# petim0/fly_bProject

Hardware: AMD Instinct MI355X
Metric: env-steps/sec (PPO rollout + update), 8192 envs per GPU (higher is better)
Workload: dtype f32 (optimizer step: fp16x2 operand split; rollout policy + critic: bf16x3 operand split; fp32 accumulate)

## Files before the change

fly_bproject_amd/csrc/fly_body.inc:

```

constexpr int LANES_PER_ENV = 8;
constexpr int BLOCK = 256;
constexpr int ENVS_PER_BLOCK = BLOCK / LANES_PER_ENV;


template <int CTRL>
__device__ __forceinline__ float dpp_f(float x)
{
    return __builtin_bit_cast(float, __builtin_amdgcn_update_dpp(0, __builtin_bit_cast(int, x), CTRL, 0xF, 0xF, true));
}
template <int CTRL>
__device__ __forceinline__ int dpp_i(int x)
{
    return __builtin_amdgcn_update_dpp(0, x, CTRL, 0xF, 0xF, true);
}
__device__ __forceinline__ float row_sum(float x)
{
    x += dpp_f<0xB1>(x);
    x += dpp_f<0x4E>(x);
    x += dpp_f<0x141>(x);
    return x;
}
__device__ __forceinline__ int row_sum_i(int x)
{
// ... 3 lines not shown
    return x;
}
__device__ __forceinline__ float row_get(float x, int src)
{
    return __shfl(x, src, LANES_PER_ENV);
}

__device__ __forceinline__ float dot3(float a0, float a1, float a2, float b0, float b1, float b2)
{
    return fmaf(a0, b0, fmaf(a1, b1, a2 * b2));
}
__device__ __forceinline__ float clampf(float x, float lim) { return fminf(fmaxf(x, -lim), lim); }

struct Root {
    float px, py, pz, qx, qy, qz, qw, vx, vy, vz, wx, wy, wz;
};

__device__ __forceinline__ void quat_rot(const float q[4], float v0, float v1, float v2, float sign, float o[3])
{
    float qw = q[3];
    float s = 2.0f * (qw * qw) - 1.0f;
    float cx = q[1] * v2 - q[2] * v1;
    float cy = q[2] * v0 - q[0] * v2;
    float cz = q[0] * v1 - q[1] * v0;
    float dot = q[0] * v0 + q[1] * v1 + q[2] * v2;
    o[0] = (v0 * s + sign * (cx * qw * 2.0f)) + q[0] * dot * 2.0f;
    o[1] = (v1 * s + sign * (cy * qw * 2.0f)) + q[1] * dot * 2.0f;
    o[2] = (v2 * s + sign * (cz * qw * 2.0f)) + q[2] * dot * 2.0f;
}

__device__ __forceinline__ float py_mod(float a, float b)
{
    float m = fmodf(a, b);
    if (m != 0.0f && ((b < 0.0f) != (m < 0.0f))) m += b;
    return m;
}

struct RootObs {
    float vl[3], wl[3], yaw, roll, pitch, ang, up_proj, heading_proj, pot;
};

__device__ __forceinline__ RootObs root_obs(const FlyConfig* __restrict__ c, const Root& r)
{
    RootObs o;
    const float two_pi = 6.28318530717958647692f;
    float t0 = c->target[0] - r.px, t1 = c->target[1] - r.py, t2 = 0.0f;
    float nrm = sqrtf(t0 * t0 + t1 * t1 + t2 * t2);
    o.pot = -nrm / c->dt;
    float dn = nrm < 1e-9f ? 1e-9f : nrm;
    float d0 = t0 / dn, d1 = t1 / dn, d2 = t2 / dn;
    float x1 = r.qx, y1 = r.qy, z1 = r.qz, w1 = r.qw;
    float x2 = -0.0f, y2 = -0.0f, z2 = -0.0f, w2 = 1.0f;
    float ww = (z1 + x1) * (x2 + y2);
    float yy = (w1 - y1) * (w2 + z2);
    float zz = (w1 + y1) * (w2 - z2);
    float xx = ww + yy + zz;
    float qq = 0.5f * (xx + (z1 - x1) * (x2 - y2));
    float tq[4];
    tq[3] = qq - ww + (z1 - y1) * (y2 - z2);
    tq[0] = qq - xx + (x1 + w1) * (x2 + w2);
    tq[1] = qq - yy + (w1 - x1) * (y2 + z2);
    tq[2] = qq - zz + (z1 + y1) * (w2 - x2);
    float up[3], hd[3];
// ... 9 lines not shown
    float roll = atan2f(sinr, cosr);
    float sinp = 2.0f * (w * y - z * x);
    float pitch;
    if (fabsf(sinp) >= 1.0f) {
        float sgn = (sinp > 0.0f) ? 1.0f : ((sinp < 0.0f) ? -1.0f : 0.0f);
        pitch = 1.57079632679489661923f * sgn;
    } else {
        pitch = asinf(sinp);
    }
    float siny = 2.0f * (w * z + x * y);
    float cosy = w * w + x * x - y * y - z * z;
    float yaw = atan2f(siny, cosy);
    o.roll = py_mod(roll, two_pi);
    o.pitch = py_mod(pitch, two_pi);
    o.yaw = py_mod(yaw, two_pi);
    float walk = atan2f(c->target[2] - r.pz, c->target[0] - r.px);
    o.ang = walk - o.yaw;
    return o;
}

__device__ __forceinline__ float scale_action(float a, float lo, float hi)
{
    float t = 0.5f * (a + 1.0f);
    t = t * (hi - lo);
    return t + lo;
}

struct FlyRegs {
    Root r;
    float jq[3], jqd[3];
    float pot, prev_pot;
    int rs;
    long progress;
    float dm[FLY_DR_PARAMS];
    uint32_t dk;
};

template <int PH, bool DR = false>
__device__ __forceinline__ void fly_load(FlyRegs& st, const FlyConfig* __restrict__ c, const FlyBuffers& b, const int block)
{
    const int n = c->num_envs;
    const int tid = threadIdx.x;
    const int sub = tid & (LANES_PER_ENV - 1);
    const long e_raw = (long)block * ENVS_PER_BLOCK + tid / LANES_PER_ENV;
    const long e = e_raw < n ? e_raw : (long)(n - 1);
    const bool is_leg = sub < FLY_NUM_LEGS;
    const int j0 = 3 * (is_leg ? sub : 0);
    constexpr bool NEED_ROOT = (PH & (PH_RESET | PH_INTEGRATE | PH_OBS | PH_REWARD)) != 0;
    constexpr bool NEED_DOF = (PH & (PH_RESET | PH_INTEGRATE | PH_OBS)) != 0;
    constexpr bool NEED_POT = (PH & (PH_RESET | PH_OBS | PH_REWARD)) != 0;
    constexpr bool NEED_FLAG = (PH & (PH_RESET | PH_REWARD)) != 0;
// ... 9 lines not shown
    for (int i = 0; i < 3; ++i) { st.jq[i] = 0.0f; st.jqd[i] = 0.0f; }
    if (NEED_DOF && is_leg) {
        const float* dp = b.dof_state + e * (FLY_NUM_DOF * 2) + 2 * j0;
#pragma unroll
        for (int i = 0; i < 3; ++i) { st.jq[i] = dp[2 * i]; st.jqd[i] = dp[2 * i + 1]; }
    }
    st.pot = 0.0f; st.prev_pot = 0.0f;
    if (NEED_POT) { st.pot = b.pot[e]; st.prev_pot = b.prev_pot[e]; }
    st.rs = 0;
    if (NEED_FLAG) st.rs = (int)(b.reset[e] != 0);
    st.progress = 0;
    if (NEED_PROG) st.progress = b.progress[e];
    if constexpr (DR && (PH & (PH_RESET | PH_INTEGRATE)) != 0) dr_load_row(c, e, st.dm, st.dk);
}

template <int PH, bool DR = false>
__device__ __forceinline__ void fly_body(const FlyConfig* __restrict__ c, const float* __restrict__ actions, const FlyBuffers& b,
                                         float* obs_tile, const int block, const FlyRegs& st, FlyRegs* st_out = nullptr,
                                         const float* actions_tile = nullptr)
{

    const int n = c->num_envs;
    const int tid = threadIdx.x;
    const int sub = tid & (LANES_PER_ENV - 1);
    const int env_in_blk = tid / LANES_PER_ENV;
    const long e_raw = (long)block * ENVS_PER_BLOCK + env_in_blk;
    const bool valid = e_raw < n;
    const long e = valid ? e_raw : (long)(n - 1);
    const bool is_leg = sub < FLY_NUM_LEGS;
    const bool is_abd = sub < FLY_NUM_ABDOMEN;
    const int leg = is_leg ? sub : 0;
    const int abd = is_abd ? sub : 0;
    const int j0 = 3 * leg;

    float lo[3], hi[3], pose[3];
#pragma unroll
    for (int i = 0; i < 3; ++i) { lo[i] = c->dof_lo[j0 + i]; hi[i] = c->dof_hi[j0 + i]; pose[i] = c->dof_pose[j0 + i]; }

    Root r = st.r;
    float jq[3] = {st.jq[0], st.jq[1], st.jq[2]}, jqd[3] = {st.jqd[0], st.jqd[1], st.jqd[2]}, jt[3] = {0, 0, 0};
    float pot = st.pot, prev_pot = st.prev_pot;
    int rs = st.rs;
    long progress = st.progress;
    float dm[FLY_DR_PARAMS];
    uint32_t dk = 0;
    bool drew = false;
    if constexpr (DR) {
#pragma unroll
        for (int j = 0; j < FLY_DR_PARAMS; ++j) dm[j] = st.dm[j];
        dk = st.dk;
    }
    float cf[3] = {0, 0, 0};
// ... 9 lines not shown
        const float* tp = b.targets + e * FLY_NUM_DOF + j0;
#pragma unroll
        for (int i = 0; i < 3; ++i) jt[i] = tp[i];
    }
    if (!(PH & (PH_INTEGRATE)) && (PH & (PH_OBS | PH_REWARD))) {
        if (is_leg) {
            const float* fp = b.contact + (e * FLY_NUM_CONTACT + FLY_NUM_ABDOMEN + leg) * 3;
            cf[0] = fp[0]; cf[1] = fp[1]; cf[2] = fp[2];
        }
        if (is_abd) {
            const float* fp = b.contact + (e * FLY_NUM_CONTACT + abd) * 3;
            cfa[0] = fp[0]; cfa[1] = fp[1]; cfa[2] = fp[2];
        }
    }

    const bool reset_after = c->reset_after_sim != 0;

    auto do_reset = [&]() {
        if (rs) {
            r.px = 0.0f; r.py = 0.0f; r.pz = c->start_height; r.qx = 0.0f; r.qy = 0.0f; r.qz = 0.0f; r.qw = 1.0f;
            r.vx = r.vy = r.vz = r.wx = r.wy = r.wz = 0.0f;
#pragma unroll
            for (int i = 0; i < 3; ++i) { jq[i] = is_leg ? pose[i] : 0.0f; jqd[i] = 0.0f; }
            float tx = c->target[0] - 0.0f, ty = c->target[1] - 0.0f;
            float nrm = sqrtf(__fadd_rn(__fadd_rn(__fmul_rn(tx, tx), __fmul_rn(ty, ty)), 0.0f));
            float p = -nrm / c->dt;
            prev_pot = p; pot = p;
            rs = 0; progress = 0;
            if constexpr (DR) {
                dr_draw(c, (uint32_t)e, dk, dm);
                dk += 1u;
                drew = true;
            }
        }
    };

    if ((PH & PH_RESET) && !(reset_after && (PH & PH_INTEGRATE))) do_reset();

    if (PH & PH_INTEGRATE) {
        const int nsub = c->substeps;
        const float h = c->dt / (float)nsub;
        const float kp = DR ? __fmul_rn(c->kp, dm[0]) : c->kp, kd = DR ? __fmul_rn(c->kd, dm[1]) : c->kd;
        const float eff = DR ? __fmul_rn(c->effort, dm[2]) : c->effort, vmax = c->vmax, Jinv = 1.0f / c->joint_inertia;
        const float minv = 1.0f / (DR ? __fmul_rn(c->mass, dm[3]) : c->mass), g = DR ? __fmul_rn(c->gravity, dm[5]) : c->gravity;
        const float I0 = DR ? __fmul_rn(c->inertia[0], dm[3]) : c->inertia[0];
        const float I1 = DR ? __fmul_rn(c->inertia[1], dm[3]) : c->inertia[1];
        const float I2 = DR ? __fmul_rn(c->inertia[2], dm[3]) : c->inertia[2];
        const float I0inv = 1.0f / I0, I1inv = 1.0f / I1, I2inv = 1.0f / I2;
        const float vlim = c->max_lin_vel, wlim = c->max_ang_vel;
        const float kc = c->kc, cd = c->cdamp, mu = DR ? __fmul_rn(c->mu, dm[4]) : c->mu, cv = c->cvisc;
        const float Lf = c->femur_len, Lt = c->tibia_len;
        const float ld = 1.0f - h * c->lin_damp, ad = 1.0f - h * c->ang_damp;
        const float att0 = c->leg_attach[leg][0], att1 = c->leg_attach[leg][1], att2 = c->leg_attach[leg][2];
        const float azim = c->leg_azimuth[leg], sg = c->leg_sigma[leg];
        const float ab0 = c->abdomen_pts[abd][0], ab1 = c->abdomen_pts[abd][1], ab2 = c->abdomen_pts[abd][2];
        const float al0 = c->alpha0, be0 = c->beta0;
        const float kc_leg = is_leg ? kc : 0.0f, kc_abd = is_abd ? kc : 0.0f;

        for (int s = 0; s < nsub; ++s) {
#pragma unroll
            for (int i = 0; i < 3; ++i) {
                float tau = fmaf(kp, jt[i] - jq[i], -(kd * jqd[i]));
                tau = fminf(fmaxf(tau, -eff), eff);
                float v = fmaf(h * Jinv, tau, jqd[i]);
                v = fminf(fmaxf(v, -vmax), vmax);
                float x = fmaf(h, v, jq[i]);
                if (x < lo[i]) { x = lo[i]; v = fmaxf(v, 0.0f); }
                if (x > hi[i]) { x = hi[i]; v = fminf(v, 0.0f); }
                jq[i] = x; jqd[i] = v;
            }
            const float qx = r.qx, qy = r.qy, qz = r.qz, qw = r.qw;
            const float R00 = fmaf(-2.0f, fmaf(qy, qy, qz * qz), 1.0f), R01 = 2.0f * fmaf(qx, qy, -(qz * qw)), R02 = 2.0f * fmaf(qx, qz, qy * qw);
            const float R10 = 2.0f * fmaf(qx, qy, qz * qw), R11 = fmaf(-2.0f, fmaf(qx, qx, qz * qz), 1.0f), R12 = 2.0f * fmaf(qy, qz, -(qx * qw));
            const float R20 = 2.0f * fmaf(qx, qz, -(qy * qw)), R21 = 2.0f * fmaf(qy, qz, qx * qw), R22 = fmaf(-2.0f, fmaf(qx, qx, qy * qy), 1.0f);
            float psi = fmaf(sg, jq[0] - pose[0], azim);
            float al = al0 + (jq[1] - pose[1]);
            float gm = al + be0 + (jq[2] - pose[2]);
            float psid = sg * jqd[0], ald = jqd[1], gmd = ald + jqd[2];
            const float sp = __sinf(psi), cp = __cosf(psi);
// ... 40 lines not shown
            float wby = dot3(R01, R11, R21, r.wx, r.wy, r.wz);
            float wbz = dot3(R02, R12, R22, r.wx, r.wy, r.wz);
            float tbx = dot3(R00, R10, R20, Tx, Ty, Tz);
            float tby = dot3(R01, R11, R21, Tx, Ty, Tz);
            float tbz = dot3(R02, R12, R22, Tx, Ty, Tz);
            float ax = (tbx - fmaf(wby * I2, wbz, -(wbz * I1 * wby))) * I0inv;
            float ay = (tby - fmaf(wbz * I0, wbx, -(wbx * I2 * wbz))) * I1inv;
            float az = (tbz - fmaf(wbx * I1, wby, -(wby * I0 * wbx))) * I2inv;
            wbx = clampf(fmaf(h, ax, wbx) * ad, wlim);
            wby = clampf(fmaf(h, ay, wby) * ad, wlim);
            wbz = clampf(fmaf(h, az, wbz) * ad, wlim);
            r.wx = dot3(R00, R01, R02, wbx, wby, wbz);
            r.wy = dot3(R10, R11, R12, wbx, wby, wbz);
            r.wz = dot3(R20, R21, R22, wbx, wby, wbz);
            r.px = fmaf(h, r.vx, r.px); r.py = fmaf(h, r.vy, r.py); r.pz = fmaf(h, r.vz, r.pz);
            const float hh = 0.5f * h;
            float nqx = fmaf(hh, fmaf(r.wx, qw, fmaf(r.wy, qz, -(r.wz * qy))), qx);
            float nqy = fmaf(hh, fmaf(-r.wx, qz, fmaf(r.wy, qw, r.wz * qx)), qy);
            float nqz = fmaf(hh, fmaf(r.wx, qy, fmaf(-r.wy, qx, r.wz * qw)), qz);
            float nqw = fmaf(hh, -fmaf(r.wx, qx, fmaf(r.wy, qy, r.wz * qz)), qw);
            float inv = __builtin_amdgcn_rsqf(fmaf(nqx, nqx, fmaf(nqy, nqy, fmaf(nqz, nqz, nqw * nqw))));
            r.qx = nqx * inv; r.qy = nqy * inv; r.qz = nqz * inv; r.qw = nqw * inv;
        }
    }

    if ((PH & PH_RESET) && reset_after && (PH & PH_INTEGRATE)) do_reset();

    float touching_f = 0.0f;
    float obs_act[3] = {0, 0, 0};
    float z_obs = 0.0f, heading_proj = 0.0f;
    if (PH & PH_OBS) {
        prev_pot = pot;
        RootObs ro = root_obs(c, r);
        pot = ro.pot;
        float* row = obs_tile + env_in_blk * FLY_NUM_OBS;
        if (sub == LANES_PER_ENV - 1) {
            row[0] = r.pz; row[1] = ro.vl[0]; row[2] = ro.vl[1]; row[3] = ro.vl[2];
            row[4] = ro.wl[0]; row[5] = ro.wl[1]; row[6] = ro.wl[2];
            row[7] = ro.yaw; row[8] = ro.roll; row[9] = ro.ang; row[10] = ro.up_proj; row[11] = ro.heading_proj;
            row[66] = ro.pitch;
        }
        z_obs = r.pz; heading_proj = ro.heading_proj;
        if (is_leg) {
            const float vs = c->dof_vel_scale;
#pragma unroll
            for (int i = 0; i < 3; ++i) {
                float u = __fsub_rn(__fsub_rn(__fmul_rn(2.0f, jq[i]), hi[i]), lo[i]) / __fsub_rn(hi[i], lo[i]);
                row[12 + j0 + i] = u;
                row[30 + j0 + i] = __fmul_rn(jqd[i], vs);
                row[48 + j0 + i] = jt[i];
                obs_act[i] = jt[i];
            }
            float ssum = __fadd_rn(__fadd_rn(cf[0], cf[1]), cf[2]);
            touching_f = ssum > 0.0f ? 1.0f : 0.0f;
            row[67 + leg] = touching_f;
        }
        __syncthreads();
        const long tile_base = (long)block * ENVS_PER_BLOCK * FLY_NUM_OBS;
        const long total = (long)n * FLY_NUM_OBS;
// ... 10 lines not shown
        }
    } else if (PH & PH_REWARD) {
        const float* row = b.obs + e * FLY_NUM_OBS;
        z_obs = row[0]; heading_proj = row[11];
        if (is_leg) {
#pragma unroll
            for (int i = 0; i < 3; ++i) obs_act[i] = row[48 + j0 + i];
        }
    }

    if (PH & PH_PROGRESS) progress += 1;

    float reward = 0.0f;
    if (PH & PH_REWARD) {
        if (progress == 0) progress = 1;
        const float uw = c->up_weight, hw = c->heading_weight;
        float elec = 0.0f, acost = 0.0f;
        int lim = 0, touching = 0;
        if (is_leg) {
#pragma unroll
            for (int i = 0; i < 3; ++i) {
                acost += jt[i] * jt[i];
                elec += fabsf(__fsub_rn(jt[i], obs_act[i]));
                lim += (obs_act[i] > __fmul_rn(hi[i], 0.9f)) ? 1 : 0;
                lim += (obs_act[i] < __fmul_rn(lo[i], 0.9f)) ? 1 : 0;
            }
            touching = (__fadd_rn(__fadd_rn(cf[0], cf[1]), cf[2]) > 0.0f) ? 1 : 0;
        }
        elec = row_sum(elec); acost = row_sum(acost);
        lim = row_sum_i(lim); touching = row_sum_i(touching);
        float bsum = is_abd ? __fadd_rn(__fadd_rn(cfa[0], cfa[1]), cfa[2]) : 0.0f;
        float abd_sum = 0.0f;
#pragma unroll
        for (int k = 0; k < FLY_NUM_ABDOMEN; ++k) abd_sum = __fadd_rn(abd_sum, row_get(bsum, k));
        const float z = z_obs;
        float heading_r = (heading_proj > 0.8f) ? hw : __fmul_rn(hw, heading_proj) / 0.8f;
        float up_r = 0.0f;
        if (z > 1.4f) up_r = __fadd_rn(up_r, uw);
        if (z < 2.1f) up_r = __fsub_rn(up_r, uw);
        float ori = __fadd_rn(__fmul_rn(r.qz, r.qz), __fmul_rn(r.qw, r.qw));
        float orient_r = (ori > 0.98f) ? uw : 0.0f;
        float leg_r = __fmul_rn((float)touching, 0.1f);
        float progress_r = __fsub_rn(pot, prev_pot);
        float total;
        if (c->reward_mode == 0) {
            total = __fadd_rn(0.5f, __fmul_rn(up_r, orient_r));
            total = __fsub_rn(total, __fmul_rn(c->energy_cost_scale, elec));
            total = __fsub_rn(total, __fmul_rn((float)lim, c->joints_at_limit_cost_scale));
            total = __fadd_rn(total, leg_r);
        } else {
            total = __fadd_rn(__fmul_rn(progress_r, 2.0f), 0.5f);
            total = __fadd_rn(total, __fmul_rn(up_r, orient_r));
            total = __fadd_rn(total, heading_r);
            total = __fsub_rn(total, __fmul_rn(c->actions_cost_scale, acost));
            total = __fsub_rn(total, __fmul_rn(c->energy_cost_scale, elec));
            total = __fsub_rn(total, __fmul_rn((float)lim, c->joints_at_limit_cost_scale));
        }
        const bool dead = (z < c->termination_height) || (z > c->termination_height_up) || (ori < 0.5f) || (abd_sum > 0.0f);
        if (dead) total = c->death_cost;
        if (dead || progress >= (long)c->max_episode_length - 1) rs = 1;
        reward = total;
    }

    if (st_out) {
        st_out->r = r;
#pragma unroll
        for (int i = 0; i < 3; ++i) { st_out->jq[i] = jq[i]; st_out->jqd[i] = jqd[i]; }
        st_out->pot = pot; st_out->prev_pot = prev_pot; st_out->rs = rs; st_out->progress = progress;
        if constexpr (DR) {
#pragma unroll
            for (int j = 0; j < FLY_DR_PARAMS; ++j) st_out->dm[j] = dm[j];
            st_out->dk = dk;
        }
    }
    if (!valid) return;
    if constexpr (DR) {
        if (drew && sub == 0) dr_store_row(c, e, dm, dk);
    }
    if (PH & (PH_SCALE)) {
        if (is_leg) {
            float* tp = b.targets + e * FLY_NUM_DOF + j0;
#pragma unroll
            for (int i = 0; i < 3; ++i) tp[i] = jt[i];
        }
    }
    if (PH & (PH_RESET | PH_INTEGRATE)) {
        if (is_leg) {
            float* dp = b.dof_state + e * (FLY_NUM_DOF * 2) + 2 * j0;
#pragma unroll
            for (int i = 0; i < 3; ++i) { dp[2 * i] = jq[i]; dp[2 * i + 1] = jqd[i]; }
        }
        if (sub == LANES_PER_ENV - 1) {
            float* rp = b.root + e * FLY_ROOT_DIM;
            rp[0] = r.px; rp[1] = r.py; rp[2] = r.pz; rp[3] = r.qx; rp[4] = r.qy; rp[5] = r.qz; rp[6] = r.qw;
            rp[7] = r.vx; rp[8] = r.vy; rp[9] = r.vz; rp[10] = r.wx; rp[11] = r.wy; rp[12] = r.wz;
        }
    }
    if (PH & PH_INTEGRATE) {
        if (is_leg) {
            float* fp = b.contact + (e * FLY_NUM_CONTACT + FLY_NUM_ABDOMEN + leg) * 3;
            fp[0] = cf[0]; fp[1] = cf[1]; fp[2] = cf[2];
        }
        if (is_abd) {
            float* fp = b.contact + (e * FLY_NUM_CONTACT + abd) * 3;
            fp[0] = cfa[0]; fp[1] = cfa[1]; fp[2] = cfa[2];
        }
    }
    if (sub == LANES_PER_ENV - 2) {
        if (PH & (PH_RESET | PH_OBS)) { b.pot[e] = pot; b.prev_pot[e] = prev_pot; }
        if (PH & (PH_RESET | PH_REWARD)) b.reset[e] = (int64_t)rs;
        if (PH & (PH_RESET | PH_REWARD | PH_PROGRESS)) b.progress[e] = (int64_t)progress;
        if (PH & PH_REWARD) {
            b.reward[e] = reward;
            if (b.ep_return) {
                const float er = b.ep_return[e] + reward, el = b.ep_length[e] + 1.0f;
                if (rs) {
                    b.done_return[e] += er; b.done_length[e] += el; b.done_count[e] += 1.0f;
                    b.ep_return[e] = 0.0f; b.ep_length[e] = 0.0f;
                } else {
                    b.ep_return[e] = er; b.ep_length[e] = el;
                }
            }
        }
    }
}
```

fly_bproject_amd/csrc/fly_env.hip:

```cpp
#include <hip/hip_runtime.h>
#include <stdint.h>
#include <type_traits>
#include "flyhip.h"
#include "domain_rand.h"
#include "launch.h"

namespace {

#include "fly_body.inc"

template <int PH>
__global__ __launch_bounds__(BLOCK) void fly_kernel(const FlyConfig* __restrict__ c,
                                                    const float* __restrict__ actions, FlyBuffers b)
{
    __shared__ __attribute__((aligned(16))) float obs_tile[ENVS_PER_BLOCK * FLY_NUM_OBS];
    FlyRegs st;
    fly_load<PH>(st, c, b, blockIdx.x);
    fly_body<PH>(c, actions, b, obs_tile, blockIdx.x, st);
}

template <int PH>
__global__ __launch_bounds__(BLOCK) void fly_dr_kernel(const FlyConfig* __restrict__ c,
                                                       const float* __restrict__ actions, FlyBuffers b)
{
    __shared__ __attribute__((aligned(16))) float obs_tile[ENVS_PER_BLOCK * FLY_NUM_OBS];
    FlyRegs st;
    fly_load<PH, true>(st, c, b, blockIdx.x);
    fly_body<PH, true>(c, actions, b, obs_tile, blockIdx.x, st);
}

inline int grid_for(int n) { return (n + ENVS_PER_BLOCK - 1) / ENVS_PER_BLOCK; }

}

extern "C" hipError_t flyhip_launch_env(int phases, const FlyConfig* dcfg, int n, const float* actions,
                                        const FlyBuffers* b, void* stream, int dr)
{
    constexpr int PH_ALL = PH_SCALE | PH_RESET | PH_INTEGRATE | PH_OBS | PH_PROGRESS | PH_REWARD;
    const dim3 grid(grid_for(n));
    if (dr && (phases & (PH_RESET | PH_INTEGRATE)))
        return with_int<PH_ALL, PH_RESET, PH_INTEGRATE>(phases, [&](auto ph) {
            return launch_kernel<fly_dr_kernel<ph.value>>(grid, BLOCK, 0, stream, dcfg, actions, *b);
        });
// ... 5 lines not shown
```

fly_bproject_amd/csrc/mlp_mfma.hip:

```cpp
#include <hip/hip_runtime.h>
#include <stdint.h>
#include <type_traits>
#include <cstdio>
#include <cstdlib>
#include "flyhip.h"
#include "mlp_layout.h"
#include "obs_norm.h"
#include "domain_rand.h"
#include "launch.h"

namespace {

#include "loss_head.inc"
#include "mlp_gemm.inc"
#include "fs_stamp.inc"
#include "mlp_forward.inc"
#include "mlp_backward.inc"
#include "mlp_grad_w.inc"
#include "mlp_fused_step.inc"
#include "mlp_adam.inc"
#include "fly_body.inc"

template <class Arith>
constexpr int RS_LDS_FLOATS = Arith::FWD_FLOATS > ENVS_PER_BLOCK * FLY_NUM_OBS ? Arith::FWD_FLOATS : ENVS_PER_BLOCK * FLY_NUM_OBS;
// ... 11 lines not shown
    typedef ArithOf<B3> Arith;
    constexpr int ARENA = RS_LDS_FLOATS<Arith>;
    __shared__ __attribute__((aligned(16))) float lds[ARENA + (NORM ? NORM_LDS_FLOATS : 0)];
    float* const norm_tab = NORM ? lds + ARENA : nullptr;
    if (NORM) obs_norm_load(norm_tab, c);
    var_steps -= var_base ? *var_base : 0;
    constexpr int PH_ALL = PH_SCALE | PH_RESET | PH_INTEGRATE | PH_OBS | PH_PROGRESS | PH_REWARD;
    FlyRegs st;
    fly_load<PH_ALL, DR>(st, c, b, blockIdx.x);
    if (NORM) __syncthreads();
    forward_body<Arith, false, false, NORM>(lds, blockIdx.x, 1L << 40, P, PF, x, n, nullptr, v_out, nullptr, nullptr, nullptr, nullptr, eps,
                                            var, act, logp, nullptr, var_steps, var_decay, var_min, norm_tab);
    __builtin_amdgcn_fence(__ATOMIC_RELEASE, "workgroup");
    __builtin_amdgcn_s_waitcnt(0);
    __syncthreads();
    fly_body<PH_ALL, DR>(c, act, b, lds, blockIdx.x, st);
}

__device__ __forceinline__ void store_pose(float* __restrict__ poses, int t, const FlyRegs& nx)
{
    const int sub = threadIdx.x;
    if (sub >= LANES_PER_ENV) return;
    float* p = poses + (long)t * FLY_POSE_FLOATS;
    if (sub < FLY_NUM_LEGS) {
#pragma unroll
        for (int i = 0; i < 3; ++i) p[7 + 3 * sub + i] = nx.jq[i];
    }
    if (sub == LANES_PER_ENV - 1) {
        p[0] = nx.r.px; p[1] = nx.r.py; p[2] = nx.r.pz; p[3] = nx.r.qx; p[4] = nx.r.qy; p[5] = nx.r.qz; p[6] = nx.r.qw;
    }
}
// ... 5 lines not shown
    float var_min, float* __restrict__ act_all, float* __restrict__ logp_all, float* __restrict__ v_ring,
    float* __restrict__ reward_all, int T, const int* __restrict__ rows_applied, int64_t* __restrict__ reset_rows,
    int64_t* __restrict__ progress_rows, float* __restrict__ poses)
{
    typedef ArithOf<B3> Arith;
    constexpr int ARENA = RS_LDS_FLOATS<Arith>;
    __shared__ __attribute__((aligned(16))) float lds[ARENA + 32 + BM * MLP_NACT + (NORM ? NORM_LDS_FLOATS : 0)];
    float* const norm_tab = NORM ? lds + ARENA + 32 + BM * MLP_NACT : nullptr;
    if (NORM) obs_norm_load(norm_tab, c);
    constexpr int PH_ALL = PH_SCALE | PH_RESET | PH_INTEGRATE | PH_OBS | PH_PROGRESS | PH_REWARD;
    float* varcur = lds + ARENA;
    float* acts = B3 ? lds + ARENA + 32 : nullptr;
    if (threadIdx.x < MLP_NACT) varcur[threadIdx.x] = var[threadIdx.x];
    FlyRegs st;
    fly_load<PH_ALL, DR>(st, c, b, blockIdx.x);
    __syncthreads();
    const bool whole = (long)(blockIdx.x + 1) * BM <= n;
    for (int t = 0; t < T; ++t) {
        const float* x = obs_ring + (long)t * n * FLY_NUM_OBS;
        float* act = act_all + (long)t * n * MLP_NACT;
        b.obs = obs_ring + (long)(t + 1) * n * FLY_NUM_OBS;
        b.reward = reward_all + (long)t * n;
        if (reset_rows) { b.reset = reset_rows + (long)t * n; b.progress = progress_rows + (long)t * n; }
        const bool in_lds = B3 && whole;
        forward_body<Arith, false, false, NORM>(lds, blockIdx.x, 1L << 40, P, PF, x, n, nullptr, v_ring + (long)t * n, nullptr, nullptr,
                                                nullptr, nullptr, eps_all + (long)t * n * MLP_NACT, varcur, act, logp_all + (long)t * n,
                                                nullptr, 0, var_decay, var_min, norm_tab, in_lds && t > 0 ? lds : nullptr,
                                                in_lds ? acts : nullptr, B3 && t > 0);
        if (!in_lds) {
            __builtin_amdgcn_fence(__ATOMIC_RELEASE, "workgroup");
            __builtin_amdgcn_s_waitcnt(0);
        }
        __syncthreads();
        FlyRegs nx;
        fly_body<PH_ALL, DR>(c, act, b, lds, blockIdx.x, st, &nx, in_lds ? acts : nullptr);
        if (REC && blockIdx.x == 0) store_pose(poses, t, nx);
        st = nx;
        if (threadIdx.x < MLP_NACT && var_decay > 0.0f) varcur[threadIdx.x] = fmaxf(var_min, varcur[threadIdx.x] - var_decay);
        if (!in_lds) asm volatile("s_waitcnt vmcnt(0)" ::: "memory");
        __syncthreads();
    }
}

template <bool STAMP, bool MULTI, bool REC, bool NORM = false, bool DR = false>
__global__ __launch_bounds__(THREADS, 1) void rollout_all_fs_kernel(
    const FlyConfig* __restrict__ c, FlyBuffers b, const float* __restrict__ P, const u16* __restrict__ PB,
    float* __restrict__ obs_ring, long n, const float* __restrict__ eps_all, const float* __restrict__ var, float var_decay,
    float var_min, float* __restrict__ act_all, float* __restrict__ logp_all, float* __restrict__ v_ring,
    float* __restrict__ reward_all, int T, int64_t* __restrict__ reset_rows, int64_t* __restrict__ progress_rows,
    void* __restrict__ aux)
{
    static_assert(!(STAMP && REC) && !(STAMP && NORM) && !(STAMP && DR), "the stamped diagnostic form neither records, normalises nor randomises");
    unsigned long long* const stamps = static_cast<unsigned long long*>(aux);
    float* const poses = static_cast<float*>(aux);
    extern __shared__ __attribute__((aligned(16))) u16 fr_lds[];
    const FrLds L(fr_lds);
    constexpr int PH_ALL = PH_SCALE | PH_RESET | PH_INTEGRATE | PH_OBS | PH_PROGRESS | PH_REWARD;
    policy_tile_fs_setup(L, P);
    float* const norm_tab = NORM ? reinterpret_cast<float*>(fr_lds) + FR_LDS_BYTES / 4 : nullptr;
    if (NORM) obs_norm_load(norm_tab, c);
    int64_t* const reset0 = b.reset;
    int64_t* const progress0 = b.progress;
    const long ntiles = n / BM;
    long tile = blockIdx.x;
    do {
        unsigned long long* st_tile = STAMP ? stamps + tile * (T + 1) * 8 : nullptr;
        if (threadIdx.x < 32) L.varcur[threadIdx.x] = threadIdx.x < MLP_NACT ? var[threadIdx.x] : 1.0f;
        b.reset = reset0; b.progress = progress0;
        FlyRegs st;
        fly_load<PH_ALL, DR>(st, c, b, (int)tile);
        WeightHeadT<2> w1;
        policy_tile_fs_head(w1, PB);
        __syncthreads();
        if (STAMP && threadIdx.x == 0) st_tile[6] = realtime_cu();
        for (int t = 0; t < T; ++t) {
            stamp<STAMP>(st_tile, 8 * t);
            float* act = act_all + (long)t * n * MLP_NACT;
            b.obs = obs_ring + (long)(t + 1) * n * FLY_NUM_OBS;
            b.reward = reward_all + (long)t * n;
            if (reset_rows) { b.reset = reset_rows + (long)t * n; b.progress = progress_rows + (long)t * n; }
            policy_tile_fs<STAMP, NORM>(L, tile, PB, t == 0 ? obs_ring : nullptr, n, v_ring + (long)t * n, eps_all + (long)t * n * MLP_NACT,
                                        act, logp_all + (long)t * n, w1, STAMP ? st_tile + 8 * t : nullptr, norm_tab);
            stamp<STAMP>(st_tile, 8 * t + 7);
            policy_tile_fs_head(w1, PB);
            FlyRegs nx;
            fly_body<PH_ALL, DR>(c, act, b, L.obs, (int)tile, st, &nx, L.acts);
            if (REC && tile == 0) store_pose(poses, t, nx);
            st = nx;
            if (threadIdx.x < MLP_NACT && var_decay > 0.0f) L.varcur[threadIdx.x] = fmaxf(var_min, L.varcur[threadIdx.x] - var_decay);
            __syncthreads();
        }
        stamp<STAMP>(st_tile, 8 * T);
        if (STAMP && threadIdx.x == 0) st_tile[8 * T + 1] = realtime_cu();
        tile += gridDim.x;
    } while (MULTI && tile < ntiles);
}

}

extern "C" hipError_t flyhip_launch_rollout_all(const FlyConfig* dcfg, const FlyBuffers* b, const float* P, const float* PF,
                                                float* obs_ring, int64_t n, const float* eps_all, const float* var,
                                                float var_decay, float var_min, float* act_all, float* logp_all, float* v_ring,
                                                float* reward_all, int T, const int* rows_applied, const uint16_t* PB,
                                                int64_t* reset_rows, int64_t* progress_rows, void* stream,
                                                unsigned long long* stamps, float* poses, int norm, int dr)
{
// ... 298 lines not shown
```

Baseline: 69.90 million.

## Keep env state and episode stats in registers across rollout steps, hoist config constants

The fused rollout kernels now carry episode return/length statistics, joint targets and contact forces in registers across all T steps, and write the physics state to global memory once at the end instead of every step. Config-derived constants (substep size, inverse masses and inertias, reward weights) are loaded once per block into a pinned register struct rather than re-read from the config pointer each step. The intent is to cut per-step global stores and loads plus scalar config reads. The cost is more register pressure, which may lower occupancy, and intermediate state buffers are no longer current during the rollout.

```diff
diff --git a/fly_bproject_amd/csrc/fly_body.inc b/fly_bproject_amd/csrc/fly_body.inc
--- a/fly_bproject_amd/csrc/fly_body.inc
+++ b/fly_bproject_amd/csrc/fly_body.inc
@@ -41,6 +41,103 @@
 
 struct Root {
     float px, py, pz, qx, qy, qz, qw, vx, vy, vz, wx, wy, wz;
+};
+
+struct FlyLane {
+    float lo[3], hi[3], pose[3];
+    int n, reset_after;
+};
+struct FlyDyn {
+    int nsub;
+    float kp, kd, effort, vmax, mass, gravity, inertia[3], mu;
+    float h, hh, hJinv, minv, Iinv[3], ld, ad;
+    float vlim, wlim, cd, cv, Lf, Lt, al0, be0;
+    float att[3], azim, sg, ab[3];
+    float kc_leg, kc_abd;
+};
+struct FlyTask {
+    int reward_mode, max_episode_length;
+    float dt, target[3], start_height, dof_vel_scale, up_weight, heading_weight;
+    float actions_cost_scale, energy_cost_scale, joints_at_limit_cost_scale, death_cost, termination_height, termination_height_up;
+};
+
+template <bool PIN>
+__device__ __forceinline__ float fly_pin(float x)
+{
+    if constexpr (PIN) asm("" : "+v"(x));
+    return x;
+}
+
+__device__ __forceinline__ void fly_lane(FlyLane& k, const FlyConfig* c, const int leg)
+{
+    const int j0 = 3 * leg;
+#pragma unroll
+    for (int i = 0; i < 3; ++i) { k.lo[i] = c->dof_lo[j0 + i]; k.hi[i] = c->dof_hi[j0 + i]; k.pose[i] = c->dof_pose[j0 + i]; }
+    k.n = c->num_envs; k.reset_after = c->reset_after_sim;
+}
+
+template <bool PIN = false>
+__device__ __forceinline__ FlyDyn fly_dyn(const FlyConfig* c, const int leg, const int abd, const bool is_leg, const bool is_abd)
+{
+    FlyDyn k;
+    auto f = [](float x) { return fly_pin<PIN>(x); };
+    k.nsub = c->substeps;
+    const float h = c->dt / (float)k.nsub, Jinv = 1.0f / c->joint_inertia;
+    k.h = f(h); k.hh = f(0.5f * h); k.hJinv = f(h * Jinv);
+    k.kp = f(c->kp); k.kd = f(c->kd); k.effort = f(c->effort); k.vmax = f(c->vmax); k.mass = f(c->mass); k.gravity = f(c->gravity);
+    k.minv = f(1.0f / c->mass);
+#pragma unroll
+    for (int i = 0; i < 3; ++i) { k.inertia[i] = f(c->inertia[i]); k.Iinv[i] = f(1.0f / c->inertia[i]); }
+    k.vlim = f(c->max_lin_vel); k.wlim = f(c->max_ang_vel);
+    const float kc = c->kc;
+    k.cd = f(c->cdamp); k.mu = f(c->mu); k.cv = f(c->cvisc);
+    k.Lf = f(c->femur_len); k.Lt = f(c->tibia_len);
+    k.ld = f(1.0f - h * c->lin_damp); k.ad = f(1.0f - h * c->ang_damp);
+#pragma unroll
+    for (int i = 0; i < 3; ++i) { k.att[i] = c->leg_attach[leg][i]; k.ab[i] = c->abdomen_pts[abd][i]; }
+    k.azim = c->leg_azimuth[leg]; k.sg = c->leg_sigma[leg];
+    k.al0 = f(c->alpha0); k.be0 = f(c->beta0);
+    k.kc_leg = is_leg ? kc : 0.0f; k.kc_abd = is_abd ? kc : 0.0f;
+    return k;
+}
+
+template <bool PIN = false>
+__device__ __forceinline__ FlyTask fly_task(const FlyConfig* c)
+{
+    FlyTask k;
+    auto f = [](float x) { return fly_pin<PIN>(x); };
+    k.reward_mode = c->reward_mode; k.max_episode_length = c->max_episode_length;
+    k.dt = f(c->dt); k.start_height = f(c->start_height);
+#pragma unroll
+    for (int i = 0; i < 3; ++i) k.target[i] = f(c->target[i]);
+    k.dof_vel_scale = f(c->dof_vel_scale); k.up_weight = f(c->up_weight); k.heading_weight = f(c->heading_weight);
+    k.actions_cost_scale = f(c->actions_cost_scale); k.energy_cost_scale = f(c->energy_cost_scale);
+    k.joints_at_limit_cost_scale = f(c->joints_at_limit_cost_scale); k.death_cost = f(c->death_cost);
+    k.termination_height = f(c->termination_height); k.termination_height_up = f(c->termination_height_up);
+    return k;
+}
+
+struct FlyRead {
+    const FlyConfig* c;
+    __device__ __forceinline__ void lane(FlyLane& k, int leg) const { fly_lane(k, c, leg); }
+    __device__ __forceinline__ FlyDyn dyn(int leg, int abd, bool is_leg, bool is_abd) const { return fly_dyn(c, leg, abd, is_leg, is_abd); }
+    __device__ __forceinline__ FlyTask task() const { return fly_task(c); }
+};
+struct FlyConsts {
+    FlyLane l;
+    FlyDyn d;
+    FlyTask t;
+    __device__ __forceinline__ explicit FlyConsts(const FlyConfig* c)
+    {
+        const int sub = threadIdx.x & (LANES_PER_ENV - 1);
+        const bool is_leg = sub < FLY_NUM_LEGS, is_abd = sub < FLY_NUM_ABDOMEN;
+        fly_lane(l, c, is_leg ? sub : 0);
+        d = fly_dyn<true>(c, is_leg ? sub : 0, is_abd ? sub : 0, is_leg, is_abd);
+        t = fly_task<true>(c);
+    }
+    __device__ __forceinline__ void lane(FlyLane& k, int) const { k = l; }
+    __device__ __forceinline__ const FlyDyn& dyn(int, int, bool, bool) const { return d; }
+    __device__ __forceinline__ const FlyTask& task() const { return t; }
 };
 
 __device__ __forceinline__ void quat_rot(const float q[4], float v0, float v1, float v2, float sign, float o[3])
@@ -67,13 +164,13 @@
     float vl[3], wl[3], yaw, roll, pitch, ang, up_proj, heading_proj, pot;
 };
 
-__device__ __forceinline__ RootObs root_obs(const FlyConfig* __restrict__ c, const Root& r)
+__device__ __forceinline__ RootObs root_obs(const FlyTask& c, const Root& r)
 {
     RootObs o;
     const float two_pi = 6.28318530717958647692f;
-    float t0 = c->target[0] - r.px, t1 = c->target[1] - r.py, t2 = 0.0f;
+    float t0 = c.target[0] - r.px, t1 = c.target[1] - r.py, t2 = 0.0f;
     float nrm = sqrtf(t0 * t0 + t1 * t1 + t2 * t2);
-    o.pot = -nrm / c->dt;
+    o.pot = -nrm / c.dt;
     float dn = nrm < 1e-9f ? 1e-9f : nrm;
     float d0 = t0 / dn, d1 = t1 / dn, d2 = t2 / dn;
     float x1 = r.qx, y1 = r.qy, z1 = r.qz, w1 = r.qw;
@@ -113,7 +210,7 @@
     o.roll = py_mod(roll, two_pi);
     o.pitch = py_mod(pitch, two_pi);
     o.yaw = py_mod(yaw, two_pi);
-    float walk = atan2f(c->target[2] - r.pz, c->target[0] - r.px);
+    float walk = atan2f(c.target[2] - r.pz, c.target[0] - r.px);
     o.ang = walk - o.yaw;
     return o;
 }
@@ -134,6 +231,66 @@
     float dm[FLY_DR_PARAMS];
     uint32_t dk;
 };
+
+struct FlyCarry {
+    float ep_return, ep_length, done_return, done_length, done_count;
+    float jt0, jt1, jt2, cf0, cf1, cf2, cfa0, cfa1, cfa2;
+};
+struct FlyNoCarry {};
+
+template <int PH>
+__device__ __forceinline__ void fly_store_state(const FlyBuffers& b, const long e, const int sub, const float (&jt)[3], const float (&jq)[3],
+                                                const float (&jqd)[3], const Root& r, const float (&cf)[3], const float (&cfa)[3])
+{
+    const bool is_leg = sub < FLY_NUM_LEGS, is_abd = sub < FLY_NUM_ABDOMEN;
+    const int leg = is_leg ? sub : 0, abd = is_abd ? sub : 0, j0 = 3 * leg;
+    if (PH & (PH_SCALE)) {
+        if (is_leg) {
+            float* tp = b.targets + e * FLY_NUM_DOF + j0;
+#pragma unroll
+            for (int i = 0; i < 3; ++i) tp[i] = jt[i];
+        }
+    }
+    if (PH & (PH_RESET | PH_INTEGRATE)) {
+        if (is_leg) {
+            float* dp = b.dof_state + e * (FLY_NUM_DOF * 2) + 2 * j0;
+#pragma unroll
+            for (int i = 0; i < 3; ++i) { dp[2 * i] = jq[i]; dp[2 * i + 1] = jqd[i]; }
+        }
+        if (sub == LANES_PER_ENV - 1) {
+            float* rp = b.root + e * FLY_ROOT_DIM;
+            rp[0] = r.px; rp[1] = r.py; rp[2] = r.pz; rp[3] = r.qx; rp[4] = r.qy; rp[5] = r.qz; rp[6] = r.qw;
+            rp[7] = r.vx; rp[8] = r.vy; rp[9] = r.vz; rp[10] = r.wx; rp[11] = r.wy; rp[12] = r.wz;
+        }
+    }
+    if (PH & PH_INTEGRATE) {
+        if (is_leg) {
+            float* fp = b.contact + (e * FLY_NUM_CONTACT + FLY_NUM_ABDOMEN + leg) * 3;
+            fp[0] = cf[0]; fp[1] = cf[1]; fp[2] = cf[2];
+        }
+        if (is_abd) {
+            float* fp = b.contact + (e * FLY_NUM_CONTACT + abd) * 3;
+            fp[0] = cfa[0]; fp[1] = cfa[1]; fp[2] = cfa[2];
+        }
+    }
+}
+
+template <int PH>
+__device__ __forceinline__ void fly_store_carried(const FlyBuffers& b, const int block, const int n, const FlyRegs& st, const FlyCarry& cy)
+{
+    const int sub = threadIdx.x & (LANES_PER_ENV - 1);
+    const long e = (long)block * ENVS_PER_BLOCK + threadIdx.x / LANES_PER_ENV;
+    if (e >= n) return;
+    const float jt[3] = {cy.jt0, cy.jt1, cy.jt2}, jq[3] = {st.jq[0], st.jq[1], st.jq[2]}, jqd[3] = {st.jqd[0], st.jqd[1], st.jqd[2]};
+    const float cf[3] = {cy.cf0, cy.cf1, cy.cf2}, cfa[3] = {cy.cfa0, cy.cfa1, cy.cfa2};
+    fly_store_state<PH>(b, e, sub, jt, jq, jqd, st.r, cf, cfa);
+    if (sub != LANES_PER_ENV - 2) return;
+    b.pot[e] = st.pot; b.prev_pot[e] = st.prev_pot;
+    if (b.ep_return) {
+        b.ep_return[e] = cy.ep_return; b.ep_length[e] = cy.ep_length;
+        b.done_return[e] = cy.done_return; b.done_length[e] = cy.done_length; b.done_count[e] = cy.done_count;
+    }
+}
 
 template <int PH, bool DR = false>
 __device__ __forceinline__ void fly_load(FlyRegs& st, const FlyConfig* __restrict__ c, const FlyBuffers& b, const int block)
@@ -173,28 +330,41 @@
     if constexpr (DR && (PH & (PH_RESET | PH_INTEGRATE)) != 0) dr_load_row(c, e, st.dm, st.dk);
 }
 
-template <int PH, bool DR = false>
-__device__ __forceinline__ void fly_body(const FlyConfig* __restrict__ c, const float* __restrict__ actions, const FlyBuffers& b,
-                                         float* obs_tile, const int block, const FlyRegs& st, FlyRegs* st_out = nullptr,
-                                         const float* actions_tile = nullptr)
-{
-
+__device__ __forceinline__ void fly_load_carry(FlyCarry& cy, const FlyConfig* __restrict__ c, const FlyBuffers& b, const int block)
+{
     const int n = c->num_envs;
+    const long e_raw = (long)block * ENVS_PER_BLOCK + threadIdx.x / LANES_PER_ENV;
+    const long e = e_raw < n ? e_raw : (long)(n - 1);
+    cy = FlyCarry{};
+    if (b.ep_return) {
+        cy.ep_return = b.ep_return[e]; cy.ep_length = b.ep_length[e];
+        cy.done_return = b.done_return[e]; cy.done_length = b.done_length[e]; cy.done_count = b.done_count[e];
+    }
+}
+
+template <int PH, bool DR = false, class Consts, class Carry = FlyNoCarry>
+__device__ __forceinline__ void fly_body(const FlyConfig* __restrict__ c, const Consts& K, const float* __restrict__ actions,
+                                         const FlyBuffers& b, float* obs_tile, const int block, const FlyRegs& st,
+                                         FlyRegs* st_out = nullptr, const float* actions_tile = nullptr, Carry* cy = nullptr)
+{
+    constexpr bool CARRY = std::is_same<Carry, FlyCarry>::value;
+
     const int tid = threadIdx.x;
     const int sub = tid & (LANES_PER_ENV - 1);
     const int env_in_blk = tid / LANES_PER_ENV;
-    const long e_raw = (long)block * ENVS_PER_BLOCK + env_in_blk;
-    const bool valid = e_raw < n;
-    const long e = valid ? e_raw : (long)(n - 1);
     const bool is_leg = sub < FLY_NUM_LEGS;
     const bool is_abd = sub < FLY_NUM_ABDOMEN;
     const int leg = is_leg ? sub : 0;
     const int abd = is_abd ? sub : 0;
     const int j0 = 3 * leg;
-
-    float lo[3], hi[3], pose[3];
-#pragma unroll
-    for (int i = 0; i < 3; ++i) { lo[i] = c->dof_lo[j0 + i]; hi[i] = c->dof_hi[j0 + i]; pose[i] = c->dof_pose[j0 + i]; }
+    FlyLane kl;
+    K.lane(kl, leg);
+    const int n = kl.n;
+    const long e_raw = (long)block * ENVS_PER_BLOCK + env_in_blk;
+    const bool valid = e_raw < n;
+    const long e = valid ? e_raw : (long)(n - 1);
+
+    const float (&lo)[3] = kl.lo, (&hi)[3] = kl.hi, (&pose)[3] = kl.pose;
 
     Root r = st.r;
     float jq[3] = {st.jq[0], st.jq[1], st.jq[2]}, jqd[3] = {st.jqd[0], st.jqd[1], st.jqd[2]}, jt[3] = {0, 0, 0};
@@ -234,17 +404,18 @@
         }
     }
 
-    const bool reset_after = c->reset_after_sim != 0;
+    const bool reset_after = kl.reset_after != 0;
 
     auto do_reset = [&]() {
         if (rs) {
-            r.px = 0.0f; r.py = 0.0f; r.pz = c->start_height; r.qx = 0.0f; r.qy = 0.0f; r.qz = 0.0f; r.qw = 1.0f;
+            const FlyTask& k = K.task();
+            r.px = 0.0f; r.py = 0.0f; r.pz = k.start_height; r.qx = 0.0f; r.qy = 0.0f; r.qz = 0.0f; r.qw = 1.0f;
             r.vx = r.vy = r.vz = r.wx = r.wy = r.wz = 0.0f;
 #pragma unroll
             for (int i = 0; i < 3; ++i) { jq[i] = is_leg ? pose[i] : 0.0f; jqd[i] = 0.0f; }
-            float tx = c->target[0] - 0.0f, ty = c->target[1] - 0.0f;
+            float tx = k.target[0] - 0.0f, ty = k.target[1] - 0.0f;
             float nrm = sqrtf(__fadd_rn(__fadd_rn(__fmul_rn(tx, tx), __fmul_rn(ty, ty)), 0.0f));
-            float p = -nrm / c->dt;
+            float p = -nrm / k.dt;
             prev_pot = p; pot = p;
             rs = 0; progress = 0;
             if constexpr (DR) {
@@ -258,31 +429,32 @@
     if ((PH & PH_RESET) && !(reset_after && (PH & PH_INTEGRATE))) do_reset();
 
     if (PH & PH_INTEGRATE) {
-        const int nsub = c->substeps;
-        const float h = c->dt / (float)nsub;
-        const float kp = DR ? __fmul_rn(c->kp, dm[0]) : c->kp, kd = DR ? __fmul_rn(c->kd, dm[1]) : c->kd;
-        const float eff = DR ? __fmul_rn(c->effort, dm[2]) : c->effort, vmax = c->vmax, Jinv = 1.0f / c->joint_inertia;
-        const float minv = 1.0f / (DR ? __fmul_rn(c->mass, dm[3]) : c->mass), g = DR ? __fmul_rn(c->gravity, dm[5]) : c->gravity;
-        const float I0 = DR ? __fmul_rn(c->inertia[0], dm[3]) : c->inertia[0];
-        const float I1 = DR ? __fmul_rn(c->inertia[1], dm[3]) : c->inertia[1];
-        const float I2 = DR ? __fmul_rn(c->inertia[2], dm[3]) : c->inertia[2];
-        const float I0inv = 1.0f / I0, I1inv = 1.0f / I1, I2inv = 1.0f / I2;
-        const float vlim = c->max_lin_vel, wlim = c->max_ang_vel;
-        const float kc = c->kc, cd = c->cdamp, mu = DR ? __fmul_rn(c->mu, dm[4]) : c->mu, cv = c->cvisc;
-        const float Lf = c->femur_len, Lt = c->tibia_len;
-        const float ld = 1.0f - h * c->lin_damp, ad = 1.0f - h * c->ang_damp;
-        const float att0 = c->leg_attach[leg][0], att1 = c->leg_attach[leg][1], att2 = c->leg_attach[leg][2];
-        const float azim = c->leg_azimuth[leg], sg = c->leg_sigma[leg];
-        const float ab0 = c->abdomen_pts[abd][0], ab1 = c->abdomen_pts[abd][1], ab2 = c->abdomen_pts[abd][2];
-        const float al0 = c->alpha0, be0 = c->beta0;
-        const float kc_leg = is_leg ? kc : 0.0f, kc_abd = is_abd ? kc : 0.0f;
+        const FlyDyn& k = K.dyn(leg, abd, is_leg, is_abd);
+        const int nsub = k.nsub;
+        const float h = k.h, hJinv = k.hJinv, hh = k.hh;
+        const float kp = DR ? __fmul_rn(k.kp, dm[0]) : k.kp, kd = DR ? __fmul_rn(k.kd, dm[1]) : k.kd;
+        const float eff = DR ? __fmul_rn(k.effort, dm[2]) : k.effort, vmax = k.vmax;
+        const float minv = DR ? 1.0f / __fmul_rn(k.mass, dm[3]) : k.minv, g = DR ? __fmul_rn(k.gravity, dm[5]) : k.gravity;
+        const float I0 = DR ? __fmul_rn(k.inertia[0], dm[3]) : k.inertia[0];
+        const float I1 = DR ? __fmul_rn(k.inertia[1], dm[3]) : k.inertia[1];
+        const float I2 = DR ? __fmul_rn(k.inertia[2], dm[3]) : k.inertia[2];
+        const float I0inv = DR ? 1.0f / I0 : k.Iinv[0], I1inv = DR ? 1.0f / I1 : k.Iinv[1], I2inv = DR ? 1.0f / I2 : k.Iinv[2];
+        const float vlim = k.vlim, wlim = k.wlim;
+        const float cd = k.cd, mu = DR ? __fmul_rn(k.mu, dm[4]) : k.mu, cv = k.cv;
+        const float Lf = k.Lf, Lt = k.Lt;
+        const float ld = k.ld, ad = k.ad;
+        const float att0 = k.att[0], att1 = k.att[1], att2 = k.att[2];
+        const float azim = k.azim, sg = k.sg;
+        const float ab0 = k.ab[0], ab1 = k.ab[1], ab2 = k.ab[2];
+        const float al0 = k.al0, be0 = k.be0;
+        const float kc_leg = k.kc_leg, kc_abd = k.kc_abd;
 
         for (int s = 0; s < nsub; ++s) {
 #pragma unroll
             for (int i = 0; i < 3; ++i) {
                 float tau = fmaf(kp, jt[i] - jq[i], -(kd * jqd[i]));
                 tau = fminf(fmaxf(tau, -eff), eff);
-                float v = fmaf(h * Jinv, tau, jqd[i]);
+                float v = fmaf(hJinv, tau, jqd[i]);
                 v = fminf(fmaxf(v, -vmax), vmax);
                 float x = fmaf(h, v, jq[i]);
                 if (x < lo[i]) { x = lo[i]; v = fmaxf(v, 0.0f); }
@@ -353,7 +525,6 @@
             r.wy = dot3(R10, R11, R12, wbx, wby, wbz);
             r.wz = dot3(R20, R21, R22, wbx, wby, wbz);
             r.px = fmaf(h, r.vx, r.px); r.py = fmaf(h, r.vy, r.py); r.pz = fmaf(h, r.vz, r.pz);
-            const float hh = 0.5f * h;
             float nqx = fmaf(hh, fmaf(r.wx, qw, fmaf(r.wy, qz, -(r.wz * qy))), qx);
             float nqy = fmaf(hh, fmaf(-r.wx, qz, fmaf(r.wy, qw, r.wz * qx)), qy);
             float nqz = fmaf(hh, fmaf(r.wx, qy, fmaf(-r.wy, qx, r.wz * qw)), qz);
@@ -370,7 +541,8 @@
     float z_obs = 0.0f, heading_proj = 0.0f;
     if (PH & PH_OBS) {
         prev_pot = pot;
-        RootObs ro = root_obs(c, r);
+        const FlyTask& k = K.task();
+        RootObs ro = root_obs(k, r);
         pot = ro.pot;
         float* row = obs_tile + env_in_blk * FLY_NUM_OBS;
         if (sub == LANES_PER_ENV - 1) {
@@ -381,7 +553,7 @@
         }
         z_obs = r.pz; heading_proj = ro.heading_proj;
         if (is_leg) {
-            const float vs = c->dof_vel_scale;
+            const float vs = k.dof_vel_scale;
 #pragma unroll
             for (int i = 0; i < 3; ++i) {
                 float u = __fsub_rn(__fsub_rn(__fmul_rn(2.0f, jq[i]), hi[i]), lo[i]) / __fsub_rn(hi[i], lo[i]);
@@ -422,7 +594,8 @@
     float reward = 0.0f;
     if (PH & PH_REWARD) {
         if (progress == 0) progress = 1;
-        const float uw = c->up_weight, hw = c->heading_weight;
+        const FlyTask& k = K.task();
+        const float uw = k.up_weight, hw = k.heading_weight;
         float elec = 0.0f, acost = 0.0f;
         int lim = 0, touching = 0;
         if (is_leg) {
@@ -451,23 +624,38 @@
         float leg_r = __fmul_rn((float)touching, 0.1f);
         float progress_r = __fsub_rn(pot, prev_pot);
         float total;
-        if (c->reward_mode == 0) {
+        if (k.reward_mode == 0) {
             total = __fadd_rn(0.5f, __fmul_rn(up_r, orient_r));
-            total = __fsub_rn(total, __fmul_rn(c->energy_cost_scale, elec));
-            total = __fsub_rn(total, __fmul_rn((float)lim, c->joints_at_limit_cost_scale));
+            total = __fsub_rn(total, __fmul_rn(k.energy_cost_scale, elec));
+            total = __fsub_rn(total, __fmul_rn((float)lim, k.joints_at_limit_cost_scale));
             total = __fadd_rn(total, leg_r);
         } else {
             total = __fadd_rn(__fmul_rn(progress_r, 2.0f), 0.5f);
             total = __fadd_rn(total, __fmul_rn(up_r, orient_r));
             total = __fadd_rn(total, heading_r);
-            total = __fsub_rn(total, __fmul_rn(c->actions_cost_scale, acost));
-            total = __fsub_rn(total, __fmul_rn(c->energy_cost_scale, elec));
-            total = __fsub_rn(total, __fmul_rn((float)lim, c->joints_at_limit_cost_scale));
-        }
-        const bool dead = (z < c->termination_height) || (z > c->termination_height_up) || (ori < 0.5f) || (abd_sum > 0.0f);
-        if (dead) total = c->death_cost;
-        if (dead || progress >= (long)c->max_episode_length - 1) rs = 1;
+            total = __fsub_rn(total, __fmul_rn(k.actions_cost_scale, acost));
+            total = __fsub_rn(total, __fmul_rn(k.energy_cost_scale, elec));
+            total = __fsub_rn(total, __fmul_rn((float)lim, k.joints_at_limit_cost_scale));
+        }
+        const bool dead = (z < k.termination_height) || (z > k.termination_height_up) || (ori < 0.5f) || (abd_sum > 0.0f);
+        if (dead) total = k.death_cost;
+        if (dead || progress >= (long)k.max_episode_length - 1) rs = 1;
         reward = total;
+    }
+
+    if constexpr (CARRY) {
+        if ((PH & PH_REWARD) && b.ep_return) {
+            const float er = cy->ep_return + reward, el = cy->ep_length + 1.0f;
+            if (rs) {
+                cy->done_return += er; cy->done_length += el; cy->done_count += 1.0f;
+                cy->ep_return = 0.0f; cy->ep_length = 0.0f;
+            } else {
+                cy->ep_return = er; cy->ep_length = el;
+            }
+        }
+        cy->jt0 = jt[0]; cy->jt1 = jt[1]; cy->jt2 = jt[2];
+        cy->cf0 = cf[0]; cy->cf1 = cf[1]; cy->cf2 = cf[2];
+        cy->cfa0 = cfa[0]; cy->cfa1 = cfa[1]; cy->cfa2 = cfa[2];
     }
 
     if (st_out) {
@@ -485,42 +673,14 @@
     if constexpr (DR) {
         if (drew && sub == 0) dr_store_row(c, e, dm, dk);
     }
-    if (PH & (PH_SCALE)) {
-        if (is_leg) {
-            float* tp = b.targets + e * FLY_NUM_DOF + j0;
-#pragma unroll
-            for (int i = 0; i < 3; ++i) tp[i] = jt[i];
-        }
-    }
-    if (PH & (PH_RESET | PH_INTEGRATE)) {
-        if (is_leg) {
-            float* dp = b.dof_state + e * (FLY_NUM_DOF * 2) + 2 * j0;
-#pragma unroll
-            for (int i = 0; i < 3; ++i) { dp[2 * i] = jq[i]; dp[2 * i + 1] = jqd[i]; }
-        }
-        if (sub == LANES_PER_ENV - 1) {
-            float* rp = b.root + e * FLY_ROOT_DIM;
-            rp[0] = r.px; rp[1] = r.py; rp[2] = r.pz; rp[3] = r.qx; rp[4] = r.qy; rp[5] = r.qz; rp[6] = r.qw;
-            rp[7] = r.vx; rp[8] = r.vy; rp[9] = r.vz; rp[10] = r.wx; rp[11] = r.wy; rp[12] = r.wz;
-        }
-    }
-    if (PH & PH_INTEGRATE) {
-        if (is_leg) {
-            float* fp = b.contact + (e * FLY_NUM_CONTACT + FLY_NUM_ABDOMEN + leg) * 3;
-            fp[0] = cf[0]; fp[1] = cf[1]; fp[2] = cf[2];
-        }
-        if (is_abd) {
-            float* fp = b.contact + (e * FLY_NUM_CONTACT + abd) * 3;
-            fp[0] = cfa[0]; fp[1] = cfa[1]; fp[2] = cfa[2];
-        }
-    }
+    if constexpr (!CARRY) fly_store_state<PH>(b, e, sub, jt, jq, jqd, r, cf, cfa);
     if (sub == LANES_PER_ENV - 2) {
-        if (PH & (PH_RESET | PH_OBS)) { b.pot[e] = pot; b.prev_pot[e] = prev_pot; }
+        if (!CARRY && (PH & (PH_RESET | PH_OBS))) { b.pot[e] = pot; b.prev_pot[e] = prev_pot; }
         if (PH & (PH_RESET | PH_REWARD)) b.reset[e] = (int64_t)rs;
         if (PH & (PH_RESET | PH_REWARD | PH_PROGRESS)) b.progress[e] = (int64_t)progress;
         if (PH & PH_REWARD) {
             b.reward[e] = reward;
-            if (b.ep_return) {
+            if (!CARRY && b.ep_return) {
                 const float er = b.ep_return[e] + reward, el = b.ep_length[e] + 1.0f;
                 if (rs) {
                     b.done_return[e] += er; b.done_length[e] += el; b.done_count[e] += 1.0f;
diff --git a/fly_bproject_amd/csrc/fly_env.hip b/fly_bproject_amd/csrc/fly_env.hip
--- a/fly_bproject_amd/csrc/fly_env.hip
+++ b/fly_bproject_amd/csrc/fly_env.hip
@@ -16,7 +16,7 @@
     __shared__ __attribute__((aligned(16))) float obs_tile[ENVS_PER_BLOCK * FLY_NUM_OBS];
     FlyRegs st;
     fly_load<PH>(st, c, b, blockIdx.x);
-    fly_body<PH>(c, actions, b, obs_tile, blockIdx.x, st);
+    fly_body<PH>(c, FlyRead{c}, actions, b, obs_tile, blockIdx.x, st);
 }
 
 template <int PH>
@@ -26,7 +26,7 @@
     __shared__ __attribute__((aligned(16))) float obs_tile[ENVS_PER_BLOCK * FLY_NUM_OBS];
     FlyRegs st;
     fly_load<PH, true>(st, c, b, blockIdx.x);
-    fly_body<PH, true>(c, actions, b, obs_tile, blockIdx.x, st);
+    fly_body<PH, true>(c, FlyRead{c}, actions, b, obs_tile, blockIdx.x, st);
 }
 
 inline int grid_for(int n) { return (n + ENVS_PER_BLOCK - 1) / ENVS_PER_BLOCK; }
diff --git a/fly_bproject_amd/csrc/mlp_mfma.hip b/fly_bproject_amd/csrc/mlp_mfma.hip
--- a/fly_bproject_amd/csrc/mlp_mfma.hip
+++ b/fly_bproject_amd/csrc/mlp_mfma.hip
@@ -49,7 +49,7 @@
     __builtin_amdgcn_fence(__ATOMIC_RELEASE, "workgroup");
     __builtin_amdgcn_s_waitcnt(0);
     __syncthreads();
-    fly_body<PH_ALL, DR>(c, act, b, lds, blockIdx.x, st);
+    fly_body<PH_ALL, DR>(c, FlyRead{c}, act, b, lds, blockIdx.x, st);
 }
 
 __device__ __forceinline__ void store_pose(float* __restrict__ poses, int t, const FlyRegs& nx)
@@ -85,6 +85,8 @@
     if (threadIdx.x < MLP_NACT) varcur[threadIdx.x] = var[threadIdx.x];
     FlyRegs st;
     fly_load<PH_ALL, DR>(st, c, b, blockIdx.x);
+    FlyCarry cy;
+    fly_load_carry(cy, c, b, blockIdx.x);
     __syncthreads();
     const bool whole = (long)(blockIdx.x + 1) * BM <= n;
     for (int t = 0; t < T; ++t) {
@@ -104,13 +106,14 @@
         }
         __syncthreads();
         FlyRegs nx;
-        fly_body<PH_ALL, DR>(c, act, b, lds, blockIdx.x, st, &nx, in_lds ? acts : nullptr);
+        fly_body<PH_ALL, DR>(c, FlyRead{c}, act, b, lds, blockIdx.x, st, &nx, in_lds ? acts : nullptr, &cy);
         if (REC && blockIdx.x == 0) store_pose(poses, t, nx);
         st = nx;
         if (threadIdx.x < MLP_NACT && var_decay > 0.0f) varcur[threadIdx.x] = fmaxf(var_min, varcur[threadIdx.x] - var_decay);
         if (!in_lds) asm volatile("s_waitcnt vmcnt(0)" ::: "memory");
         __syncthreads();
     }
+    if (T > 0) fly_store_carried<PH_ALL>(b, blockIdx.x, (int)n, st, cy);
 }
 
 template <bool STAMP, bool MULTI, bool REC, bool NORM = false, bool DR = false>
@@ -133,6 +136,7 @@
     int64_t* const reset0 = b.reset;
     int64_t* const progress0 = b.progress;
     const long ntiles = n / BM;
+    const FlyConsts k(c);
     long tile = blockIdx.x;
     do {
         unsigned long long* st_tile = STAMP ? stamps + tile * (T + 1) * 8 : nullptr;
@@ -140,6 +144,8 @@
         b.reset = reset0; b.progress = progress0;
         FlyRegs st;
         fly_load<PH_ALL, DR>(st, c, b, (int)tile);
+        FlyCarry cy;
+        fly_load_carry(cy, c, b, (int)tile);
         WeightHeadT<2> w1;
         policy_tile_fs_head(w1, PB);
         __syncthreads();
@@ -155,12 +161,13 @@
             stamp<STAMP>(st_tile, 8 * t + 7);
             policy_tile_fs_head(w1, PB);
             FlyRegs nx;
-            fly_body<PH_ALL, DR>(c, act, b, L.obs, (int)tile, st, &nx, L.acts);
+            fly_body<PH_ALL, DR>(c, k, act, b, L.obs, (int)tile, st, &nx, L.acts, &cy);
             if (REC && tile == 0) store_pose(poses, t, nx);
             st = nx;
             if (threadIdx.x < MLP_NACT && var_decay > 0.0f) L.varcur[threadIdx.x] = fmaxf(var_min, L.varcur[threadIdx.x] - var_decay);
             __syncthreads();
         }
+        if (T > 0) fly_store_carried<PH_ALL>(b, (int)tile, (int)n, st, cy);
         stamp<STAMP>(st_tile, 8 * T);
         if (STAMP && threadIdx.x == 0) st_tile[8 * T + 1] = realtime_cu();
         tile += gridDim.x;
```

Result: faster. 70.69 million, median of 6 (+1.1%).
